# pzimbrod/fem-glass-tempering

Hardware: AMD Instinct MI355X
Metric: DOF-updates/sec (coupled thermo-visco time step, 3D CG1 hex) (higher is better)
Workload: dtype f64; 1 GPU; C4 3D plate CG1/CG1 400x400x50 hex (8200851 T-dofs), dt 0.1, coupled 6-term Prony; parallelism=single GPU, one partition (no communication), output=none (reference writes VTX/XDMF every step), krylov_form=PETSc KSPCG, geometric-multigrid V-cycle preconditioner, preconditioner=gmg, visco_fields=state (T, Tf, Tf_partial, phi, xi, s_tilde, sigma_tilde, sigma)

## Files before the change

fem-glass-tempering_amd/csrc/tv_cg.hip:

```cpp
#include <algorithm>
#include <cstdlib>

#include "tv_stencil.h"


#include <cstdio>
#include <vector>

namespace tv {
namespace {


using buf_t = __amdgpu_buffer_rsrc_t;
using b64v = unsigned int __attribute__((ext_vector_type(2)));
constexpr uint32_t kBadOff = 0x40000000u;
__device__ __forceinline__ buf_t mk_rsrc(const void* p, uint32_t bytes) {
  const uint64_t a = (uint64_t)p;
  const uint32_t lo = __builtin_amdgcn_readfirstlane((uint32_t)a);
  const uint32_t hi = __builtin_amdgcn_readfirstlane((uint32_t)(a >> 32));
  void* q = (void*)(((uint64_t)hi << 32) | lo);
  return __builtin_amdgcn_make_buffer_rsrc(q, (short)0, (int)__builtin_amdgcn_readfirstlane(bytes), 0x00020000);
}
__device__ __forceinline__ double bload(buf_t r, uint32_t off) {
  return __builtin_bit_cast(double, __builtin_amdgcn_raw_buffer_load_b64(r, (int)off, 0, 0));
// ... 274 lines not shown
  double Tp[3][3], Pp[3][3];
#pragma unroll
  for (int u = 0; u < 3; ++u)
#pragma unroll
    for (int v = 0; v < 3; ++v) {
      const int a = c[t1] + u - 1, b = c[t2] + v - 1;
      const bool ok = a >= 0 && a < n[t1] && b >= 0 && b < n[t2];
      const int64_t off = me + (int64_t)(u - 1) * st[t1] + (int64_t)(v - 1) * st[t2];
      if (MODE == MODE_RES) {
        Tp[u][v] = ok ? in0[off] : 0.0;
        Pp[u][v] = 0.0;
      } else {
        Tp[u][v] = ok ? T[off] : 0.0;
        double pv = ok ? in0[off] : 0.0;
        if (FUSEP && ok && !first) pv = pv + bcoef * pold[off];
        Pp[u][v] = pv;
      }
    }
  const double* c1 = g.coef[t1] + (int64_t)c[t1] * C_NCOEF;
  const double* c2 = g.coef[t2] + (int64_t)c[t2] * C_NCOEF;
  return facet_sum<MODE, false, false, false>(g, c1[C_HLO], c1[C_HHI], c2[C_HLO], c2[C_HHI], Tp, Pp);
}

struct FaceOff {
  int off[7];
};

FaceOff face_offsets(const CgGrid& g, int R, int qaxis) {
  FaceOff fo{};
  int acc = 0;
  const int rows = R - 1;
  for (int f = 0; f < 6; ++f) {
    fo.off[f] = acc;
    if (g.fface[f] && (f >> 1) != qaxis) acc += ((g.fn1[f] + kSeg - 1) / kSeg) * ((g.fn2[f] + rows - 1) / rows);
  }
  fo.off[6] = acc;
  return fo;
}

__device__ __forceinline__ void facet_corners(const CgGrid& g, bool ok, double h1, double h2, double Ta,
                                              double Tc, double Pa, double Pc, double& ya, double& yb,
                                              double& yc, double& yd) {
  const double Tb = shl1(Ta), Td = shl1(Tc), Pb = shl1(Pa), Pd = shl1(Pc);
  ya = yb = yc = yd = 0.0;
  if (ok) {
#pragma unroll
    for (int q1 = 0; q1 < 3; ++q1) {
#pragma unroll
      for (int q2 = 0; q2 < 3; ++q2) {
        const double sx = kGX[q1], tx = kGX[q2];
        const double fa = (1.0 - sx) * (1.0 - tx), fb = sx * (1.0 - tx), fc = (1.0 - sx) * tx, fd = sx * tx;
        const double Th = fa * Ta + fb * Tb + fc * Tc + fd * Td;
        const double Ph = fa * Pa + fb * Pb + fc * Pc + fd * Pd;
        const double G = (kGW[q1] * kGW[q2]) * dg_rad_conv(g, Th) * Ph;
        ya += G * fa;
        yb += G * fb;
        yc += G * fc;
        yd += G * fd;
      }
    }
    const double sc = g.dt * (h1 * h2);
    ya *= sc; yb *= sc; yc *= sc; yd *= sc;
  }
}

template <bool FUSEP, int R>
__device__ void face_block(const CgGrid& g, const double* __restrict__ T, const double* __restrict__ in0,
                           const double* pA, const double* pB, double beta_ratio,
                           double* __restrict__ partials, const RedTail& rt, int nrec, int fb,
                           const FaceOff& fo, double* sm, double* redf, int it_host) {
  double (*sT)[kWave] = reinterpret_cast<double (*)[kWave]>(sm);
  double (*sP)[kWave] = reinterpret_cast<double (*)[kWave]>(sm + (R + 1) * kWave);
  double (*sCD)[R][kWave] = reinterpret_cast<double (*)[R][kWave]>(sm + 2 * (R + 1) * kWave);
  int f = 0;
  while (f < 5 && fb >= fo.off[f + 1]) ++f;
  const int a = f >> 1, side = f & 1;
  const int t1 = (a == 0) ? 1 : 0, t2 = (a == 2) ? 1 : 2;
  const int n[3] = {g.n0, g.n1, g.n2};
  const int sst[3] = {1, g.n0, g.n0 * g.n1};
  const int n1 = n[t1], n2 = n[t2];
  const int nseg1 = (n1 + kSeg - 1) / kSeg;
  const int tile = fb - fo.off[f];
  const int seg = tile % nseg1, tb = tile / nseg1;
  const int lane = threadIdx.x & (kWave - 1);
  const int wave = __builtin_amdgcn_readfirstlane(threadIdx.x >> 6);
  const int c1 = seg * kSeg - 1 + lane;
  const int r0 = tb * (R - 1);
// ... 1249 lines not shown
                             hipStream_t s) {
  if (!use_march(g) || !g.bnodes || g.n_bnodes <= 0) return false;
  launch_rows<MODE_RES, false>(g, T, T, Tp, F, nullptr, nullptr, nullptr, false, s, nullptr, 0, true, dinv);
  return true;
}

void launch_cg_japply(const CgGrid& g, const double* T, const double* x, double* y, double* partials,
                      int* n_partials, hipStream_t s, const PcgState* st) {
  launch_rows<MODE_JAC, false>(g, T, x, nullptr, y, nullptr, st, partials, false, s);
  if (n_partials) *n_partials = plan(g, false).nparts;
}

bool launch_cg_japply_tail(const CgGrid& g, const double* T, const double* x, double* y, const PcgState* st,
                           double* partials, const RedTail* tail, hipStream_t s) {
  return launch_rows<MODE_JAC, false>(g, T, x, nullptr, y, nullptr, st, partials, false, s, tail, 0, true);
}

void launch_cg_facet_faces(const CgGrid& g, const double* T, const double* x, const PcgState* st, hipStream_t s) {
  const FaceOff fo = face_offsets(g, kRows, -1);
  if (fo.off[6] <= 0) return;
  hipLaunchKernelGGL(k_cg_faces_all<kRows>, dim3(fo.off[6]), dim3(kRows * kWave), 0, s, g, T, x, fo, st);
}

FaceAdd cg_face_add_all(const CgGrid& g) {
  FaceAdd fa = cg_face_add(g, 0);
  if (!fa.on) return fa;
  for (int f = 0; f < 6; ++f) fa.ff[f] = g.fface[f];
  return fa;
}

void launch_cg_japply_partial(const CgGrid& g, const double* T, const double* x, double* y, const PcgState* st,
                              hipStream_t s) {
  launch_rows<MODE_JAC, false>(g, T, x, nullptr, y, nullptr, st, nullptr, false, s, nullptr, 0, false);
}

bool launch_cg_japply_fused(const CgGrid& g, const double* T, const double* z, double* pA, double* pB,
                            double* w, const PcgState* st, double* partials, int* n_partials,
                            hipStream_t s, const RedTail* tail, int it_host) {
  if (tail && tail->lag && tail->lag_kind != 3) return false;
  const bool fused = launch_rows<MODE_JAC, true>(g, T, z, pA, w, pB, st, partials, true, s, tail, it_host);
  if (n_partials) *n_partials = plan(g, true).nparts;
  return fused;
}

bool launch_cg_cgs(const CgGrid& g, bool init, const CgsBuffers& v, PcgState* st, double* partials,
                   hipStream_t s, const RedTail* tail, int it_host, const double* lag_sums) {
// ... 41 lines not shown
```

fem-glass-tempering_amd/csrc/tv_ctx.h:

```cpp
#pragma once
#include <rccl/rccl.h>

#include <algorithm>
#include <array>
#include <cmath>
#include <cstdio>
#include <cstring>
#include <memory>
#include <mutex>
#include <string>
#include <vector>

#include "tv_internal.h"

namespace tv {

struct FieldInfo {
  double* ptr = nullptr;
  void* base = nullptr;
  int bs = 1;
  int space = 0;
  bool alloc = false;
};

// ... 60 lines not shown
  int64_t globT_off = 0, globS_off = 0;
  int mixed_part = 0;
  int64_t outT_n = 0, outS_n = 0;
  std::vector<std::vector<double>> coords;
  FieldInfo f[TV_NUM_FIELDS];
  double* coef[3] = {nullptr, nullptr, nullptr};
  double* dgh[3] = {nullptr, nullptr, nullptr};
  int* map = nullptr;
  int64_t* bnodes = nullptr;
  double* ffbuf[2] = {nullptr, nullptr};
  double *r = nullptr, *z = nullptr, *pA = nullptr, *pB = nullptr, *w = nullptr, *dinv = nullptr;
  bool cgs = false;
  bool dir_on = false;
  double dir_value = 0.0;
  double *dB = nullptr, *dtmp = nullptr;
  double* Tfo = nullptr;
  int relaxation = TV_RELAX_TAYLOR;
  Output* out = nullptr;
  bool mg_on = false;
  bool mg_dg = false;
  std::vector<MgLevel> mg;
  double mg_omega0 = 0.0;
  double* mgx = nullptr;
  bool mg_cgs = false;
  double* mg_s = nullptr;
  double* dggface = nullptr;
  int mg_A = 0;
  bool mg_local = false;
  double* mg_mask0 = nullptr;
  double* h_big = nullptr;
  size_t h_big_n = 0;
  bool um = false;
  UmGrid umg{};
  std::vector<double> um_xyz;
  std::vector<int64_t> um_cells;
  UmDevice* umd = nullptr;
  unsigned char* um_bmask = nullptr;
  bool amg_on = false;
  std::vector<AmgLevel> amg;
  std::vector<void*> amg_bufs;
  int64_t um_own_cells = 0;
  std::vector<int> um_peer;
  std::vector<int64_t> um_rcnt, um_roff, um_scnt, um_soff;
  int64_t* um_sidx = nullptr;
  double* um_sbuf = nullptr;
  std::vector<int> out_fields;
// ... 120 lines not shown
  int ts_reserve;
  bool ahead;
};
using KrylovIterate = int (*)(void* f, int it, int b, int nb);
using KrylovPublished = int (*)(void* f);
int krylov_drive(Ctx* c, const KrylovPolicy& p, KrylovIterate iterate, void* fi, KrylovPublished published, void* fp,
                 int* its, int* reason);
template <class Iterate, class Published>
int krylov_drive(Ctx* c, const KrylovPolicy& p, Iterate iterate, Published published, int* its, int* reason) {
  return krylov_drive(
      c, p, [](void* f, int it, int b, int nb) -> int { return (*static_cast<Iterate*>(f))(it, b, nb); }, &iterate,
      [](void* f) -> int { return (*static_cast<Published*>(f))(); }, &published, its, reason);
}
CgsBuffers cgs_buffers(Ctx* c, const double* T, int it);
int newton(Ctx* c, int* out_its, int* out_kits, int* out_conv, int step_end = 0, bool* end_queued = nullptr);
int visco(Ctx* c, bool copy_Tprev, const NewtonGate& gate = NewtonGate{});
int queue_newton_norm(Ctx* c, const double* nrm2);
int publish(Ctx* c, void* host_dst, const void* dev_src, size_t bytes);
void launch_bc_mask(Ctx* c, double* dinv);

int mg_setup(Ctx* c);
int mg_prepare(Ctx* c, const double* T);
int mg_dg_weight(Ctx* c, const double* T);
int mg_apply0(Ctx* c, const double* T, const RedTail* tail);
int pcg_solve_mg(Ctx* c, const double* T, int* its, int* reason, bool post = false);
KrylovPolicy mg_krylov_policy(Ctx* c);
bool mg_next_level(const std::vector<double> (&Xp)[3], double da, bool automatic, std::vector<double> (&Xc)[3],
                   std::vector<char> (&is_c)[3], int coarse[3]);
void mg_axis_tables(const std::vector<double>& Xf, const std::vector<char>& is_c, std::vector<int>& pi,
                    std::vector<double>& pw, std::vector<int>& ri, std::vector<double>& rw);
int mg_level_vectors(Ctx* c, MgLevel& L);
double mg_gershgorin(const std::vector<double> (&X)[3], double dt_alpha);
double mg_omega(double b);
int mg_level(Ctx* c, size_t l);
template <class T>
int mg_upload(Ctx* c, MgLevel& L, const std::vector<T>& h, const T** out) {
  void* p = nullptr;
  HIPC(tv_dev_alloc(&p, sizeof(T) * std::max<size_t>(1, h.size()), mem_kind<T>()));
  L.bufs.push_back(p);
  HIPC(hipMemcpy(p, h.data(), sizeof(T) * h.size(), hipMemcpyHostToDevice));
  *out = static_cast<const T*>(p);
  return TV_OK;
}

int mg_setup_dist(Ctx* c);
int pcg_solve_mg_dist(Ctx* c, const double* T, int* its, int* reason, bool post = false);
int mg_prepare_dist(Ctx* c, const double* T);
// ... 5 lines not shown
```

fem-glass-tempering_amd/csrc/tv_internal.h:

```cpp
#pragma once
#include <hip/hip_runtime.h>
#include <cstdint>
#include <string>
#include <type_traits>
#include <vector>

#include "tvfem.h"

namespace tv {

constexpr int kWave = 64;
constexpr int kSeg = kWave - 2;
constexpr int kBlock = 256;

enum { kMemDoubles = 0, kMemOther = 1 };
template <class T>
constexpr int mem_kind() {
  return std::is_same<T, double>::value ? kMemDoubles : kMemOther;
}
hipError_t tv_dev_alloc(void** p, size_t bytes, int kind);
hipError_t tv_dev_free(void* p);
template <class T>
inline hipError_t tv_dev_alloc(T** p, size_t bytes, int kind) {
  void* q = nullptr;
// ... 273 lines not shown
  const double* T_amb;
  const double* eps;
  const int* probes;
  double* hist;
};
void launch_ensemble(const EnsArgs& a, const ViscoConst& c, const ViscoFields& f, const EnsExt* x, hipStream_t s);
void launch_ensemble_dg(const EnsArgs& a, const ViscoConst& c, const ViscoFields& f, const EnsExt* x, hipStream_t s);

constexpr int kVecBlocks = 1024;
constexpr int kVecBlocksMin = 256;
constexpr int kVecNodesPerThread = 16;
constexpr int kVecBlocksMax = 8192;
void launch_pcg_init(int64_t n, const double* r, const double* dinv, double* z, double* dx,
                     double* partials, hipStream_t s);
struct FaceAdd {
  int on;
  int n0, n1, n2;
  int64_t t_off;
  double inv_n0, inv_plane;
  const double* ff[6];
};
FaceAdd cg_face_add(const CgGrid& g, int64_t t_off);


struct MgXfer {
  int fn[3], cn[3];
  int coarse[3];
  int f_kb, f_ke, c_kb, c_ke;
  const int* pi[3];
  const double* pw[3];
  const int* ri[3];
  const double* rw[3];
  int aligned;
};
void launch_mg_restrict(const MgXfer& x, const PcgState* st, const double* bf, const double* wf, const FaceAdd* fa,
                        const double* mask, double* bc, const double* dinv_c, double omega_c, double* xc,
                        hipStream_t s);
struct RRAxis {
  const int* f0;
  const double* w;
};
struct RRArgs {
  int on;
  int fn[3], cn[3];
  RRAxis ax[3];
  double da;
// ... 30 lines not shown
  MgXfer xf[kMgPrepMax];
  double* T[kMgPrepMax];
  double* dinv[kMgPrepMax];
  CgGrid g[kMgPrepMax];
  int64_t off_n[kMgPrepMax + 1];
  int64_t off_b[kMgPrepMax + 1];
};
void launch_mg_prepare(const MgPrep& p, hipStream_t s);
bool cg_uses_march(const CgGrid& g);
void launch_mg_dg_restrict(const DgGrid& g, const PcgState* st, const double* bf, const double* wf, const double* mask,
                           double* bc, const double* dinv_c, double omega_c, double* xc, int kg0, hipStream_t s);
void launch_mg_dg_prolong(const DgGrid& g, const PcgState* st, double* xf, const double* xc, const double* mask,
                          int kg0, hipStream_t s);
void launch_mg_dg_T(const DgGrid& g, const double* Tdg, double* Tcg, int kg0, hipStream_t s);
int launch_mg_pow(int64_t n, const double* dinv, double* y, double* partials, hipStream_t s);
void launch_mg_scale(int64_t n, const double* y, double a, double* x, hipStream_t s);
bool launch_cg_japply_tail(const CgGrid& g, const double* T, const double* x, double* y, const PcgState* st,
                           double* partials, const RedTail* tail, hipStream_t s);
void launch_cg_japply_partial(const CgGrid& g, const double* T, const double* x, double* y, const PcgState* st,
                              hipStream_t s);
void launch_mg_update(int64_t n, const PcgState* st, const double* pA, const double* pB, const double* w,
                      const FaceAdd* fa, const double* dinv, double omega, double* r, double* dx, double* x0,
                      int it_host, int init, hipStream_t s, const double* lag = nullptr,
                      unsigned* counter = nullptr);
void launch_mg_update_cgs(int64_t n, const PcgState* st, const double* u, double* s, const double* z, double* p,
                          double* dx, double* r, const double* dinv, double omega, double* x0, bool first,
                          const double* lag, int lag_kind, unsigned* counter, hipStream_t stream);
int launch_cg_japply_post(const CgGrid& g, const double* T, const double* x, const double* r, const double* dinv,
                          double omega, double* z, const PcgState* st, double* partials, const RedTail* tail,
                          hipStream_t s);
int launch_mg_post(int64_t n, const PcgState* st, const double* x0, const double* r, const double* w,
                   const FaceAdd* fa, const double* dinv, double omega, double* z, double* partials,
                   const RedTail* tail, hipStream_t s);

void launch_pcg_update(int64_t n, PcgState* st, const double* pA, const double* pB, const double* w,
                       const double* dinv, double* dx, double* z, double* partials, hipStream_t s,
                       const RedTail* tail = nullptr, const FaceAdd* fa = nullptr, int it_host = 0);
void launch_pcg_dx_tail(int64_t n, const PcgState* st, const double* pA, const double* pB, double* dx, int its,
                        hipStream_t s);
void launch_mg_dx_finish(int64_t n, const PcgState* st, const double* pA, const double* pB, double* dx, int its,
                         hipStream_t s);
void launch_reduce_logic(const double* partials, int n, int W, double* out, PcgState* st, int kind,
                         int check_done, hipStream_t s);
void launch_logic(PcgState* st, const double* sums, int kind, hipStream_t s);
void launch_set_state(PcgState* st, const PcgState& h, hipStream_t s, const double* gate = nullptr);
void launch_newton_update(int64_t n, double* T, const double* dx, double* partials, hipStream_t s,
                          const RedTail* tail = nullptr);
// ... 22 lines not shown
```

fem-glass-tempering_amd/csrc/tv_mgsolve.cpp:

```cpp
#include <cstdlib>

#include "tv_ctx.h"

namespace tv {
constexpr int64_t kMgFoldFacesNodes = 4000000;

double mg_gershgorin(const std::vector<double> (&X)[3], double dt_alpha) {
  using Row = std::array<double, 6>;
  std::vector<Row> rows[3];
  for (int s = 0; s < 3; ++s) {
    std::vector<double> cf;
    axis_coefs(X[s], 0, (int)X[s].size(), cf);
    for (size_t i = 0; i < X[s].size(); ++i) {
      const double* c = &cf[i * C_NCOEF];
      rows[s].push_back({c[C_MLO], c[C_MDI], c[C_MUP], c[C_KLO], c[C_KDI], c[C_KUP]});
    }
    std::sort(rows[s].begin(), rows[s].end());
    rows[s].erase(std::unique(rows[s].begin(), rows[s].end()), rows[s].end());
  }
  double b = 0.0;
  for (const Row& r0 : rows[0])
    for (const Row& r1 : rows[1])
      for (const Row& r2 : rows[2]) {
        double sum = 0.0, diag = 0.0;
// ... 281 lines not shown
    std::vector<double> rw[3];
    for (int s = 0; s < 3; ++s) {
      std::vector<int> pi;
      std::vector<double> pw;
      mg_axis_tables(Xp[s], is_c[s], pi, pw, ri[s], rw[s]);
      if (int e = mg_upload(c, L, pi, &x.pi[s])) return e;
      if (int e = mg_upload(c, L, pw, &x.pw[s])) return e;
      if (int e = mg_upload(c, L, ri[s], &x.ri[s])) return e;
      if (int e = mg_upload(c, L, rw[s], &x.rw[s])) return e;
      x.fn[s] = (int)Xp[s].size();
      x.cn[s] = (int)L.X[s].size();
      x.coarse[s] = coarse[s];
    }
    x.f_kb = 0;
    x.f_ke = x.fn[2];
    x.c_kb = 0;
    x.c_ke = x.cn[2];
    x.aligned = 1;
    const size_t from = c->mg.size() - 1 - (dg ? 1 : 0);
    if (!dg && ((rr_levels(c->nT) >> from) & 1u))
      if (int e = rr_setup(c, L, Xp, ri, rw)) return e;
    for (int s = 0; s < 3; ++s) Xp[s] = L.X[s];
  }
  c->mg_on = true;
  return TV_OK;
}


int mg_prepare(Ctx* c, const double* T) {
  if (c->amg_on) return TV_OK;
  const bool dgpart = c->mg_dg && c->n_parts > 1;
  auto dg_T = [&](MgLevel& L) -> int {
    if (!dgpart) {
      launch_mg_dg_T(c->dg, T, L.T, 0, c->stream);
      return TV_OK;
    }
    HIPC(hipMemsetAsync(L.T, 0, sizeof(double) * (size_t)L.n, c->stream));
    launch_mg_dg_T(c->dg, T, L.T, c->plane_begin - c->dg.k_begin, c->stream);
    return allreduce_vec(c, L.T, L.n);
  };
  const size_t base = c->mg_dg ? 1 : 0;
  const size_t ncg = c->mg.size() - std::min(c->mg.size(), base);
  bool ready = ncg > 0 && ncg <= (size_t)kMgPrepMax;
  for (size_t l = base; l < c->mg.size() && ready; ++l)
    ready = c->mg[l].dinv_interior && cg_uses_march(c->mg[l].g) && c->mg[l].g.bnodes != nullptr;
  if (ready) {
    if (base == 1) {
      MgLevel& L = c->mg[0];
// ... 50 lines not shown
  if (l < c->mg.size()) {
    const MgLevel& C = c->mg[l];
    const FaceAdd fa = cg_face_add(L.g, 0);
    if (C.rr.on && fa.on) {
      launch_cg_facet_faces(L.g, L.T, L.x, c->st, s);
      if (!launch_mg_rrestrict(C.rr, c->st, L.b, L.x, cg_face_add_all(L.g), C.b, C.dinv, C.omega, C.x, s))
        return c->fail(TV_ERR_STATE, kRRChunkMsg);
    } else if (fa.on && mg_restrict_folds_faces(C.xf)) {
      launch_cg_japply_partial(L.g, L.T, L.x, L.w, c->st, s);
      launch_mg_restrict(C.xf, c->st, L.b, L.w, &fa, nullptr, C.b, C.dinv, C.omega, C.x, s);
    } else {
      launch_cg_japply(L.g, L.T, L.x, L.w, nullptr, nullptr, s, c->st);
      launch_mg_restrict(C.xf, c->st, L.b, L.w, nullptr, nullptr, C.b, C.dinv, C.omega, C.x, s);
    }
    if (int e = mg_level(c, l + 1)) return e;
    mg_prolong_from(c, l, L.x, nullptr);
    launch_cg_japply_partial(L.g, L.T, L.x, L.w, c->st, s);
    if (!mg_prolong_smooths(L.xf))
      launch_mg_jacobi(L.n, c->st, L.b, L.w, &fa, L.dinv, L.omega, L.x, 1, s);
  }
  return TV_OK;
}

int mg_apply0(Ctx* c, const double* T, const RedTail* tail) {
  if (c->amg_on) return amg_apply0(c, tail);
  const int64_t n = c->nT;
  hipStream_t s = c->stream;
  const double* mask = c->dir_on ? c->dinv : nullptr;
  if (c->mg_dg) {
    const DgGrid& d = c->dg;
    MgLevel& C = c->mg[0];
    if (c->n_parts > 1) {
      const int kg0 = c->plane_begin - d.k_begin;
      if (int e = halo(c, c->mgx)) return -e;
      launch_dg_japply(d, T, c->mgx, c->w, nullptr, nullptr, s, c->st);
      if (hipMemsetAsync(C.b, 0, sizeof(double) * (size_t)C.n, s) != hipSuccess)
        return -c->fail(TV_ERR_HIP, "GMG: level-1 memset");
      launch_mg_dg_restrict(d, c->st, c->r, c->w, mask, C.b, nullptr, 0.0, nullptr, kg0, s);
      if (int e = allreduce_vec(c, C.b, C.n)) return -e;
      launch_mg_jacobi(C.n, c->st, C.b, nullptr, nullptr, C.dinv, C.omega, C.x, 0, s);
      if (int e = mg_level(c, 1)) return -e;
      launch_mg_dg_prolong(d, c->st, c->mgx, C.x, mask, kg0, s);
    } else {
      launch_dg_japply(d, T, c->mgx, c->w, nullptr, nullptr, s, c->st);
      launch_mg_dg_restrict(d, c->st, c->r, c->w, mask, C.b, C.dinv, C.omega, C.x, 0, s);
      if (int e = mg_level(c, 1)) return -e;
      launch_mg_dg_prolong(d, c->st, c->mgx, C.x, mask, 0, s);
    }
    launch_dg_japply(d, T, c->mgx, c->w, nullptr, nullptr, s, c->st);
    if (c->dggface)
      return launch_dg_bpost(d, c->st, c->mgx, c->r, c->w, c->dggface, c->mg_omega0, c->z, c->partials, tail, s);
    return launch_mg_post(n, c->st, c->mgx, c->r, c->w, nullptr, c->dinv, c->mg_omega0, c->z, c->partials, tail, s);
  }
  const FaceAdd fa = cg_face_add(c->cg, 0);
  if (!c->mg.empty()) {
    MgLevel& C = c->mg[0];
    if (C.rr.on && mask == nullptr && fa.on) {
      launch_cg_facet_faces(c->cg, T, c->mgx, c->st, s);
      if (!launch_mg_rrestrict(C.rr, c->st, c->r, c->mgx, cg_face_add_all(c->cg), C.b, C.dinv, C.omega, C.x, s))
        return -c->fail(TV_ERR_STATE, kRRChunkMsg);
    } else if (fa.on && mg_restrict_folds_faces(C.xf) && n < kMgFoldFacesNodes) {
      launch_cg_japply_partial(c->cg, T, c->mgx, c->w, c->st, s);
      launch_mg_restrict(C.xf, c->st, c->r, c->w, &fa, mask, C.b, C.dinv, C.omega, C.x, s);
    } else {
      launch_cg_japply(c->cg, T, c->mgx, c->w, nullptr, nullptr, s, c->st);
      launch_mg_restrict(C.xf, c->st, c->r, c->w, nullptr, mask, C.b, C.dinv, C.omega, C.x, s);
    }
    if (int e = mg_level(c, 1)) return -e;
    mg_prolong_from(c, 0, c->mgx, mask);
  }
  {
    const int nrec = launch_cg_japply_post(c->cg, T, c->mgx, c->r, c->dinv, c->mg_omega0, c->z, c->st, c->partials,
                                           tail, s);
    if (nrec >= 0) return nrec;
  }
  launch_cg_japply_partial(c->cg, T, c->mgx, c->w, c->st, s);
  return launch_mg_post(n, c->st, c->mgx, c->r, c->w, &fa, c->dinv, c->mg_omega0, c->z, c->partials, tail, s);
}

int mg_iteration(Ctx* c, const double* T, int it) {
  const int64_t n = c->nT;
  RedTail t1{c->counters, c->partials, c->sums, c->st, 2, iter_stamp(c, it)};
  int np = 0;
  if (!op_japply_fused(c, T, &np, &t1, it))
    if (int e = reduce_logic(c, np, 1, 2, 1)) return e;
  const FaceAdd fa = (c->mg_dg || c->um) ? FaceAdd{} : cg_face_add(c->cg, 0);
  if (c->dggface)
    launch_dg_bupdate(c->dg, c->st, c->pA, c->pB, c->w, c->dggface, c->mg_omega0, c->r, c->f[TV_F_DX].ptr, c->mgx, it, 0,
                      c->stream);
  else
    launch_mg_update(n, c->st, c->pA, c->pB, c->w, &fa, c->dinv, c->mg_omega0, c->r, c->f[TV_F_DX].ptr, c->mgx, it, 0,
                     c->stream);
  RedTail t2{c->counters + kTailCounters, c->partials, c->sums, c->st, 3, nullptr};
  const int nrec = mg_apply0(c, T, &t2);
  return nrec < 0 ? -nrec : TV_OK;
}

KrylovPolicy mg_krylov_policy(Ctx* c) {
  KrylovPolicy p{};
  p.ahead = false;
  p.hints = c->mg_hint;
  p.hint_min = 0;
  p.first_default = 1;
  p.hint_floor = 1;
  p.next = 1;
  p.guard = c->O.ksp_max_it + 2;
  p.ts_reserve = c->O.ksp_max_it + 8;
  return p;
}

int pcg_solve_mg(Ctx* c, const double* T, int* its, int* reason, bool post) {
  const int64_t n = c->nT;
  solve_begin(c, c->solve_gate);
  if (int e = mg_prepare(c, T)) return e;
  if (int e = mg_dg_weight(c, T)) return e;
  if (c->dggface)
    launch_dg_bupdate(c->dg, c->st, c->pA, c->pB, c->w, c->dggface, c->mg_omega0, c->r, c->f[TV_F_DX].ptr, c->mgx, 0, 1,
                      c->stream);
  else
    launch_mg_update(n, c->st, c->pA, c->pB, c->w, nullptr, c->dinv, c->mg_omega0, c->r, c->f[TV_F_DX].ptr, c->mgx, 0, 1,
                     c->stream);
  RedTail t0{c->counters + kTailCounters, c->partials, c->sums, c->st, 1, nullptr};
  if (const int nrec = mg_apply0(c, T, &t0); nrec < 0) return -nrec;
  auto iterate = [&](int it, int, int) { return mg_iteration(c, T, it); };
  auto published = [&]() -> int {
    if (!post) return TV_OK;
    launch_post_group(n, c->st, c->pA, c->pB, c->f[TV_F_DX].ptr, c->f[TV_F_T].ptr, c->partials, c->sums, c->stream);
    return queue_newton_norm(c, c->sums);
  };
  if (int e = krylov_drive(c, mg_krylov_policy(c), iterate, published, its, reason)) return e;
  if (!post) launch_mg_dx_finish(n, c->st, c->pA, c->pB, c->f[TV_F_DX].ptr, *its, c->stream);
  return TV_OK;
}

}

using namespace tv;

static int precond_apply_part(Ctx* c, const double* r_dev, double* z_dev) {
  if (int e = require_comm(c, "tv_precond_apply")) return e;
  if (c->um || c->fam_T != TV_CG) return c->fail(TV_ERR_ARG, "tv_precond_apply: partitioned CG1 box meshes");
  const double* T = c->f[TV_F_T].ptr;
  const int64_t off = c->ownT_off, n = c->ownT_n;
  hipStream_t s = c->stream;
  if (int e = halo(c, c->f[TV_F_T].ptr)) return e;
  launch_cg_diag(c->cg, T, c->dinv, 1, s, c->dinv_interior);
// ... 4 lines not shown
  } else {
    PcgState h{};
    HIPC(hipMemcpyAsync(c->st, &h, sizeof(PcgState), hipMemcpyHostToDevice, s));
    if (int e = mg_prepare_dist(c, T)) return e;
    if (c->dir_on)
      if (int e = halo(c, c->dinv)) return e;
    if (c->mg_mask0) launch_mg_ownmask(c->nT, off, off + n, c->dir_on ? c->dinv : nullptr, c->mg_mask0, s);
    HIPC(hipMemcpyAsync(c->r + off, r_dev, sizeof(double) * (size_t)n, hipMemcpyDeviceToDevice, s));
    int64_t woff, nwin;
    fine_window(c, &woff, &nwin);
    if (c->ghost_depth > 1)
      if (int e = halo(c, c->r)) return e;
    launch_mg_jacobi(nwin, c->st, c->r + woff, nullptr, nullptr, c->dinv + woff, c->mg_omega0, c->mgx + woff, 0, s);
    if (int e = mg_apply0_dist(c, T, nullptr)) return e;
    HIPC(hipMemcpyAsync(z_dev, c->z + off, sizeof(double) * (size_t)n, hipMemcpyDeviceToDevice, s));
  }
  HIPC(hipGetLastError());
  HIPC(hipStreamSynchronize(s));
  return TV_OK;
}

extern "C" {

int tv_precond_apply(void* ctx, const double* r_dev, double* z_dev) {
  Ctx* c = static_cast<Ctx*>(ctx);
  if (!c || !r_dev || !z_dev) return TV_ERR_ARG;
  hipSetDevice(c->device);
  HIPC(hipDeviceSynchronize());
  if (c->n_parts > 1) return precond_apply_part(c, r_dev, z_dev);
  const double* T = c->f[TV_F_T].ptr;
  const int64_t n = c->nT;
  hipStream_t s = c->stream;
  if (!c->dggface) {
    if (!c->um && c->fam_T == TV_CG) {
      launch_cg_diag(c->cg, T, c->dinv, 1, s, c->dinv_interior);
      c->dinv_interior = true;
    } else {
      op_diag(c, T, c->dinv, 1);
    }
  }
  if (c->dir_on && c->fam_T == TV_CG) launch_bc_mask(c, c->dinv);
  if (c->mg_dg || c->amg_on)
    if (int e = mg_dg_weight(c, T)) return e;
  if (!c->mg_on) {
    launch_mg_jacobi(n, nullptr, r_dev, nullptr, nullptr, c->dinv, 1.0, z_dev, 0, s);
  } else {
// ... 18 lines not shown
```

fem-glass-tempering_amd/csrc/tv_pcg.hip:

```cpp
#include <algorithm>
#include <cstdlib>

#include "tv_device.h"

namespace tv {
namespace {

__device__ __forceinline__ double wave_sum(double v) {
#pragma unroll
  for (int off = 32; off >= 1; off >>= 1) v += __shfl_xor(v, off, 64);
  return v;
}

template <int W>
__device__ __forceinline__ void block_partials(double (&v)[W], double* partials) {
  __shared__ double red[W][kBlock / kWave];
  const int lane = threadIdx.x & 63, wave = threadIdx.x >> 6;
#pragma unroll
  for (int w = 0; w < W; ++w) {
    const double s = wave_sum(v[w]);
    if (lane == 0) red[w][wave] = s;
  }
  __syncthreads();
  if (threadIdx.x < W) {
    const int w = threadIdx.x;
    store_partial(&partials[(int64_t)blockIdx.x * W + w], (red[w][0] + red[w][1]) + (red[w][2] + red[w][3]));
// ... 66 lines not shown
      v[4] = ldc<NT1>(&pp[q]);
      v[5] = p[q];
    }
  };
  constexpr int U = 4;
  const int64_t stride = (int64_t)gridDim.x * kBlock;
  int64_t t = blockIdx.x * (int64_t)kBlock + threadIdx.x;
  for (; t + (U - 1) * stride < n; t += U * stride) {
    double v[U][6];
#pragma unroll
    for (int u = 0; u < U; ++u) load(t + u * stride, v[u]);
#pragma unroll
    for (int u = 0; u < U; ++u) node(t + u * stride, v[u]);
  }
  for (; t < n; t += stride) {
    double v[6];
    load(t, v);
    node(t, v);
  }
  block_partials<2>(acc, partials);
  fused_reduce_tail<2>(rt, gridDim.x);
}

template <bool FACES, bool INIT, bool DXU, bool FIRST = false>
__global__ __launch_bounds__(kBlock) void k_mg_update(int64_t n, const PcgState* __restrict__ st,
                                                      const double* __restrict__ pA, const double* __restrict__ pB,
                                                      const double* __restrict__ w, FaceAdd fa,
                                                      const double* __restrict__ dinv, double omega,
                                                      double* __restrict__ r, double* __restrict__ dx,
                                                      double* __restrict__ x0, int it_host, const double* lag,
                                                      unsigned* counter, PcgState* st_w) {
  double a = 0.0, ap = 0.0;
  if (!INIT && lag != nullptr) {
    const PcgState ls = lagged_state(st, lag, 2);
    if (ls.done) { commit_done(st_w, ls); return; }
    a = ls.a;
    ap = DXU ? ls.a_prev : 0.0;
  } else {
    if (st->done) return;
    a = INIT ? 0.0 : st->a;
    ap = DXU ? st->a_prev : 0.0;
  }
  const double* __restrict__ p = (it_host & 1) ? pB : pA;
  const double* __restrict__ pp = (it_host & 1) ? pA : pB;
  auto load = [&](int64_t q, double (&v)[6]) {
    v[0] = r[q];
    v[2] = ldc<true>(&dinv[q]);
    if (!INIT) v[1] = ldc<true>(&w[q]);
    if (DXU) {
      v[3] = FIRST ? 0.0 : ldc<true>(&dx[q]);
      v[4] = ldc<true>(&pp[q]);
      v[5] = ldc<true>(&p[q]);
    }
  };
  auto node = [&](int64_t q, const double (&v)[6]) {
    double rr = v[0];
    if (INIT) {
    } else {
      double wt = v[1];
      if (FACES) wt += face_terms(fa, q);
      rr -= a * wt;
      r[q] = rr;
      if (DXU) stc<true>(&dx[q], (v[3] + ap * v[4]) + a * v[5]);
    }
    x0[q] = omega * v[2] * rr;
  };
  constexpr int U = 4;
  const int64_t stride = (int64_t)gridDim.x * kBlock;
  int64_t t = blockIdx.x * (int64_t)kBlock + threadIdx.x;
  for (; t + (U - 1) * stride < n; t += U * stride) {
    double v[U][6];
#pragma unroll
    for (int u = 0; u < U; ++u) load(t + u * stride, v[u]);
#pragma unroll
    for (int u = 0; u < U; ++u) node(t + u * stride, v[u]);
  }
  for (; t < n; t += stride) {
    double v[6];
    load(t, v);
    node(t, v);
  }
  if (!INIT && lag != nullptr && last_block_arrived(counter, gridDim.x) && threadIdx.x == 0) {
    const PcgState ls = lagged_state(st, lag, 2);
    *st_w = ls;
  }
}

template <bool FIRST>
__global__ __launch_bounds__(kBlock) void k_mg_update_cgs(int64_t n, const PcgState* __restrict__ st,
                                                          const double* __restrict__ u, double* __restrict__ s,
                                                          const double* __restrict__ z, double* __restrict__ p,
                                                          double* __restrict__ dx, double* __restrict__ r,
// ... 174 lines not shown
__global__ __launch_bounds__(kBlock) void k_copy(double* __restrict__ d, const double* __restrict__ s, int64_t n) {
  for (int64_t t = blockIdx.x * (int64_t)kBlock + threadIdx.x; t < n; t += (int64_t)gridDim.x * kBlock) d[t] = s[t];
}

int vec_blocks(int64_t n) {
  int64_t b = (n + kBlock - 1) / kBlock;
  const int64_t lim = std::min<int64_t>(kVecBlocks, std::max<int64_t>(kVecBlocksMin,
      (n + (int64_t)kBlock * kVecNodesPerThread - 1) / ((int64_t)kBlock * kVecNodesPerThread)));
  if (b > lim) b = lim;
  return b < 1 ? 1 : (int)b;
}

}

int pcg_vec_blocks(int64_t n) { return vec_blocks(n); }

void launch_pcg_init(int64_t n, const double* r, const double* dinv, double* z, double* dx, double* partials,
                     hipStream_t s) {
  hipLaunchKernelGGL(k_pcg_init, dim3(vec_blocks(n)), dim3(kBlock), 0, s, n, r, dinv, z, dx, partials);
}

void launch_mg_update(int64_t n, const PcgState* st, const double* pA, const double* pB, const double* w,
                      const FaceAdd* fa, const double* dinv, double omega, double* r, double* dx, double* x0,
                      int it_host, int init, hipStream_t s, const double* lag, unsigned* counter) {
  const FaceAdd f = (fa && fa->on) ? *fa : FaceAdd{};
  const dim3 g(vec_blocks(n)), b(kBlock);
  const bool odd = (it_host & 1) != 0;
  const bool first = it_host == 1;
#define TV_MGU(F, I, D, FI) \
  hipLaunchKernelGGL((k_mg_update<F, I, D, FI>), g, b, 0, s, n, st, pA, pB, w, f, dinv, omega, r, dx, x0, it_host, \
                     lag, counter, const_cast<PcgState*>(st))
  if (init) TV_MGU(false, true, false, false);
  else if (f.on) {
    if (first) TV_MGU(true, false, true, true);
    else if (odd) TV_MGU(true, false, true, false);
    else TV_MGU(true, false, false, false);
  } else {
    if (first) TV_MGU(false, false, true, true);
    else if (odd) TV_MGU(false, false, true, false);
    else TV_MGU(false, false, false, false);
  }
#undef TV_MGU
}

int launch_mg_post(int64_t n, const PcgState* st, const double* x0, const double* r, const double* w,
                   const FaceAdd* fa, const double* dinv, double omega, double* z, double* partials,
                   const RedTail* tail, hipStream_t s) {
  const RedTail rt = tail ? *tail : RedTail{};
  const FaceAdd f = (fa && fa->on) ? *fa : FaceAdd{};
  const int nb = vec_blocks(n);
  if (f.on)
    hipLaunchKernelGGL(k_mg_post<true>, dim3(nb), dim3(kBlock), 0, s, n, st, x0, r, w, f, dinv, omega, z, partials, rt);
  else
    hipLaunchKernelGGL(k_mg_post<false>, dim3(nb), dim3(kBlock), 0, s, n, st, x0, r, w, f, dinv, omega, z, partials, rt);
// ... 98 lines not shown
```

fem-glass-tempering_amd/csrc/tv_stencil.h:

```cpp
#pragma once
#include "tv_device.h"

namespace tv {
namespace {

enum { MODE_RES = 0, MODE_JAC = 1 };

__device__ constexpr double kGX[3] = {0.11270166537925831148, 0.5, 0.88729833462074168852};
__device__ constexpr double kGW[3] = {5.0 / 18.0, 8.0 / 18.0, 5.0 / 18.0};

__device__ __forceinline__ double g_rad_conv(const CgGrid& g, double T) {
  const double T2 = T * T;
  return g.a_rad * (T2 * T2 - g.T_amb4) + g.a_conv * (T - g.T_amb);
}
__device__ __forceinline__ double dg_rad_conv(const CgGrid& g, double T) {
  return g.a_rad * 4.0 * (T * T * T) + g.a_conv;
}

template <int MODE, bool DIAG, bool D1, bool D2>
__device__ double facet_sum(const CgGrid& g, double h1lo, double h1hi, double h2lo, double h2hi,
                            const double (&Tp)[3][3], const double (&Pp)[3][3]) {
  double acc = 0.0;
  constexpr int NS1 = D1 ? 1 : 2, NQ1 = D1 ? 1 : 3;
  constexpr int NS2 = D2 ? 1 : 2, NQ2 = D2 ? 1 : 3;
#pragma unroll
  for (int s1 = 0; s1 < NS1; ++s1) {
    const double h1 = D1 ? 1.0 : (s1 == 0 ? h1lo : h1hi);
    if (!D1 && !(h1 > 0.0)) continue;
    const int o1 = D1 ? 0 : (s1 == 0 ? -1 : 1);
#pragma unroll
    for (int s2 = 0; s2 < NS2; ++s2) {
      const double h2 = D2 ? 1.0 : (s2 == 0 ? h2lo : h2hi);
      if (!D2 && !(h2 > 0.0)) continue;
      const int o2 = D2 ? 0 : (s2 == 0 ? -1 : 1);
      const double T00 = Tp[1][1], T10 = Tp[1 + o1][1], T01 = Tp[1][1 + o2], T11 = Tp[1 + o1][1 + o2];
      const double P00 = Pp[1][1], P10 = Pp[1 + o1][1], P01 = Pp[1][1 + o2], P11 = Pp[1 + o1][1 + o2];
#pragma unroll
      for (int q1 = 0; q1 < NQ1; ++q1) {
        const double pc1 = D1 ? 1.0 : (s1 == 0 ? kGX[q1] : 1.0 - kGX[q1]);
// ... 65 lines not shown
```

Baseline: 846.7 million DOF-updates/s.

## Fold boundary-facet Jacobian of x0 into the MG update kernel

Extra blocks are appended to the multigrid update kernel. Each one recomputes the updated residual and the Jacobi x0 on boundary faces and evaluates the radiation/convection facet contribution of x0 into a face buffer. This removes the separate launch_cg_facet_faces kernel and its reread of r, dinv and T on the faces before restriction. It caches face residuals, dinv and T in double-buffered face arrays, adds four face-sized allocations, and duplicates the residual update on face nodes.

```diff
diff --git a/fem-glass-tempering_amd/csrc/tv_cg.hip b/fem-glass-tempering_amd/csrc/tv_cg.hip
--- a/fem-glass-tempering_amd/csrc/tv_cg.hip
+++ b/fem-glass-tempering_amd/csrc/tv_cg.hip
@@ -320,10 +320,6 @@
   return facet_sum<MODE, false, false, false>(g, c1[C_HLO], c1[C_HHI], c2[C_HLO], c2[C_HHI], Tp, Pp);
 }
 
-struct FaceOff {
-  int off[7];
-};
-
 FaceOff face_offsets(const CgGrid& g, int R, int qaxis) {
   FaceOff fo{};
   int acc = 0;
@@ -336,31 +332,6 @@
   return fo;
 }
 
-__device__ __forceinline__ void facet_corners(const CgGrid& g, bool ok, double h1, double h2, double Ta,
-                                              double Tc, double Pa, double Pc, double& ya, double& yb,
-                                              double& yc, double& yd) {
-  const double Tb = shl1(Ta), Td = shl1(Tc), Pb = shl1(Pa), Pd = shl1(Pc);
-  ya = yb = yc = yd = 0.0;
-  if (ok) {
-#pragma unroll
-    for (int q1 = 0; q1 < 3; ++q1) {
-#pragma unroll
-      for (int q2 = 0; q2 < 3; ++q2) {
-        const double sx = kGX[q1], tx = kGX[q2];
-        const double fa = (1.0 - sx) * (1.0 - tx), fb = sx * (1.0 - tx), fc = (1.0 - sx) * tx, fd = sx * tx;
-        const double Th = fa * Ta + fb * Tb + fc * Tc + fd * Td;
-        const double Ph = fa * Pa + fb * Pb + fc * Pc + fd * Pd;
-        const double G = (kGW[q1] * kGW[q2]) * dg_rad_conv(g, Th) * Ph;
-        ya += G * fa;
-        yb += G * fb;
-        yc += G * fc;
-        yd += G * fd;
-      }
-    }
-    const double sc = g.dt * (h1 * h2);
-    ya *= sc; yb *= sc; yc *= sc; yd *= sc;
-  }
-}
 
 template <bool FUSEP, int R>
 __device__ void face_block(const CgGrid& g, const double* __restrict__ T, const double* __restrict__ in0,
@@ -1656,6 +1627,8 @@
   hipLaunchKernelGGL(k_cg_faces_all<kRows>, dim3(fo.off[6]), dim3(kRows * kWave), 0, s, g, T, x, fo, st);
 }
 
+FaceOff cg_face_offsets_all(const CgGrid& g, int R) { return face_offsets(g, R, -1); }
+
 FaceAdd cg_face_add_all(const CgGrid& g) {
   FaceAdd fa = cg_face_add(g, 0);
   if (!fa.on) return fa;
diff --git a/fem-glass-tempering_amd/csrc/tv_ctx.h b/fem-glass-tempering_amd/csrc/tv_ctx.h
--- a/fem-glass-tempering_amd/csrc/tv_ctx.h
+++ b/fem-glass-tempering_amd/csrc/tv_ctx.h
@@ -106,6 +106,8 @@
   std::vector<MgLevel> mg;
   double mg_omega0 = 0.0;
   double* mgx = nullptr;
+  double* rfbuf[4] = {nullptr, nullptr, nullptr, nullptr};
+  bool mg_fold_ok = false, mg_fold = false;
   bool mg_cgs = false;
   double* mg_s = nullptr;
   double* dggface = nullptr;
@@ -272,7 +274,7 @@
 int mg_setup(Ctx* c);
 int mg_prepare(Ctx* c, const double* T);
 int mg_dg_weight(Ctx* c, const double* T);
-int mg_apply0(Ctx* c, const double* T, const RedTail* tail);
+int mg_apply0(Ctx* c, const double* T, const RedTail* tail, bool x0_faces = false);
 int pcg_solve_mg(Ctx* c, const double* T, int* its, int* reason, bool post = false);
 KrylovPolicy mg_krylov_policy(Ctx* c);
 bool mg_next_level(const std::vector<double> (&Xp)[3], double da, bool automatic, std::vector<double> (&Xc)[3],
diff --git a/fem-glass-tempering_amd/csrc/tv_internal.h b/fem-glass-tempering_amd/csrc/tv_internal.h
--- a/fem-glass-tempering_amd/csrc/tv_internal.h
+++ b/fem-glass-tempering_amd/csrc/tv_internal.h
@@ -319,6 +319,23 @@
 };
 FaceAdd cg_face_add(const CgGrid& g, int64_t t_off);
 
+struct FaceOff {
+  int off[7];
+};
+FaceOff cg_face_offsets_all(const CgGrid& g, int R);
+
+struct MgFold {
+  int on;
+  CgGrid g;
+  const double* T;
+  FaceOff fo;
+  const double* rold[6];
+  double* rnew[6];
+  double* xface[6];
+  double* tface[6];
+  double* dface[6];
+};
+
 
 struct MgXfer {
   int fn[3], cn[3];
@@ -395,7 +412,7 @@
 void launch_mg_update(int64_t n, const PcgState* st, const double* pA, const double* pB, const double* w,
                       const FaceAdd* fa, const double* dinv, double omega, double* r, double* dx, double* x0,
                       int it_host, int init, hipStream_t s, const double* lag = nullptr,
-                      unsigned* counter = nullptr);
+                      unsigned* counter = nullptr, const MgFold* fold = nullptr);
 void launch_mg_update_cgs(int64_t n, const PcgState* st, const double* u, double* s, const double* z, double* p,
                           double* dx, double* r, const double* dinv, double omega, double* x0, bool first,
                           const double* lag, int lag_kind, unsigned* counter, hipStream_t stream);
diff --git a/fem-glass-tempering_amd/csrc/tv_mgsolve.cpp b/fem-glass-tempering_amd/csrc/tv_mgsolve.cpp
--- a/fem-glass-tempering_amd/csrc/tv_mgsolve.cpp
+++ b/fem-glass-tempering_amd/csrc/tv_mgsolve.cpp
@@ -327,8 +327,41 @@
       if (int e = rr_setup(c, L, Xp, ri, rw)) return e;
     for (int s = 0; s < 3; ++s) Xp[s] = L.X[s];
   }
+  const char* fe = std::getenv("TVFEM_MG_FOLD");
+  const bool fold_env = !(fe && std::atoi(fe) == 0);
+  if (!dg && fold_env && c->n_parts == 1 && !c->mg.empty() && c->mg[0].rr.on && cg_face_add(c->cg, 0).on &&
+      c->cg.ffsize > 0 && c->cg.ffbuf[1] != nullptr) {
+    for (int q = 0; q < 4; ++q) {
+      void* p = nullptr;
+      HIPC(tv_dev_alloc(&p, sizeof(double) * (size_t)c->cg.ffsize, kMemDoubles));
+      HIPC(hipMemsetAsync(p, 0, sizeof(double) * (size_t)c->cg.ffsize, c->stream));
+      c->mg[0].bufs.push_back(p);
+      c->rfbuf[q] = static_cast<double*>(p);
+    }
+    c->mg_fold_ok = true;
+  }
   c->mg_on = true;
   return TV_OK;
+}
+
+static MgFold mg_fold_args(Ctx* c, const double* T, int it, bool init) {
+  MgFold m{};
+  if (!c->mg_fold) return m;
+  m.on = 1;
+  m.g = c->cg;
+  m.T = T;
+  m.fo = cg_face_offsets_all(c->cg, kBlock / kWave);
+  const int ro = init ? 0 : (it & 1), wn = init ? 0 : ((it + 1) & 1);
+  for (int f = 0; f < 6; ++f) {
+    const int64_t off = c->cg.ffoff[f];
+    if (off < 0 || !c->cg.fface[f]) continue;
+    m.rold[f] = c->rfbuf[ro] + off;
+    m.rnew[f] = c->rfbuf[wn] + off;
+    m.xface[f] = c->cg.ffbuf[1] + off;
+    m.tface[f] = c->rfbuf[2] + off;
+    m.dface[f] = c->rfbuf[3] + off;
+  }
+  return m;
 }
 
 
@@ -425,7 +458,7 @@
   return TV_OK;
 }
 
-int mg_apply0(Ctx* c, const double* T, const RedTail* tail) {
+int mg_apply0(Ctx* c, const double* T, const RedTail* tail, bool x0_faces) {
   if (c->amg_on) return amg_apply0(c, tail);
   const int64_t n = c->nT;
   hipStream_t s = c->stream;
@@ -459,8 +492,14 @@
   if (!c->mg.empty()) {
     MgLevel& C = c->mg[0];
     if (C.rr.on && mask == nullptr && fa.on) {
-      launch_cg_facet_faces(c->cg, T, c->mgx, c->st, s);
-      if (!launch_mg_rrestrict(C.rr, c->st, c->r, c->mgx, cg_face_add_all(c->cg), C.b, C.dinv, C.omega, C.x, s))
+      FaceAdd fx = cg_face_add_all(c->cg);
+      if (x0_faces) {
+        for (int f = 0; f < 6; ++f)
+          if (fx.ff[f]) fx.ff[f] = c->cg.ffbuf[1] + c->cg.ffoff[f];
+      } else {
+        launch_cg_facet_faces(c->cg, T, c->mgx, c->st, s);
+      }
+      if (!launch_mg_rrestrict(C.rr, c->st, c->r, c->mgx, fx, C.b, C.dinv, C.omega, C.x, s))
         return -c->fail(TV_ERR_STATE, kRRChunkMsg);
     } else if (fa.on && mg_restrict_folds_faces(C.xf) && n < kMgFoldFacesNodes) {
       launch_cg_japply_partial(c->cg, T, c->mgx, c->w, c->st, s);
@@ -491,11 +530,13 @@
   if (c->dggface)
     launch_dg_bupdate(c->dg, c->st, c->pA, c->pB, c->w, c->dggface, c->mg_omega0, c->r, c->f[TV_F_DX].ptr, c->mgx, it, 0,
                       c->stream);
-  else
+  else {
+    const MgFold fold = mg_fold_args(c, T, it, false);
     launch_mg_update(n, c->st, c->pA, c->pB, c->w, &fa, c->dinv, c->mg_omega0, c->r, c->f[TV_F_DX].ptr, c->mgx, it, 0,
-                     c->stream);
+                     c->stream, nullptr, nullptr, &fold);
+  }
   RedTail t2{c->counters + kTailCounters, c->partials, c->sums, c->st, 3, nullptr};
-  const int nrec = mg_apply0(c, T, &t2);
+  const int nrec = mg_apply0(c, T, &t2, c->mg_fold);
   return nrec < 0 ? -nrec : TV_OK;
 }
 
@@ -517,14 +558,17 @@
   solve_begin(c, c->solve_gate);
   if (int e = mg_prepare(c, T)) return e;
   if (int e = mg_dg_weight(c, T)) return e;
+  c->mg_fold = c->mg_fold_ok && !c->dir_on && !c->amg_on && !c->mg_dg;
   if (c->dggface)
     launch_dg_bupdate(c->dg, c->st, c->pA, c->pB, c->w, c->dggface, c->mg_omega0, c->r, c->f[TV_F_DX].ptr, c->mgx, 0, 1,
                       c->stream);
-  else
+  else {
+    const MgFold fold = mg_fold_args(c, T, 0, true);
     launch_mg_update(n, c->st, c->pA, c->pB, c->w, nullptr, c->dinv, c->mg_omega0, c->r, c->f[TV_F_DX].ptr, c->mgx, 0, 1,
-                     c->stream);
+                     c->stream, nullptr, nullptr, &fold);
+  }
   RedTail t0{c->counters + kTailCounters, c->partials, c->sums, c->st, 1, nullptr};
-  if (const int nrec = mg_apply0(c, T, &t0); nrec < 0) return -nrec;
+  if (const int nrec = mg_apply0(c, T, &t0, c->mg_fold); nrec < 0) return -nrec;
   auto iterate = [&](int it, int, int) { return mg_iteration(c, T, it); };
   auto published = [&]() -> int {
     if (!post) return TV_OK;
@@ -575,6 +619,14 @@
 
 extern "C" {
 
+int tv_mg_update_faces(void* ctx, int* in_force, int* set_up) {
+  Ctx* c = static_cast<Ctx*>(ctx);
+  if (!c || !in_force || !set_up) return TV_ERR_ARG;
+  *in_force = c->mg_fold ? 1 : 0;
+  *set_up = c->mg_fold_ok ? 1 : 0;
+  return TV_OK;
+}
+
 int tv_precond_apply(void* ctx, const double* r_dev, double* z_dev) {
   Ctx* c = static_cast<Ctx*>(ctx);
   if (!c || !r_dev || !z_dev) return TV_ERR_ARG;
diff --git a/fem-glass-tempering_amd/csrc/tv_pcg.hip b/fem-glass-tempering_amd/csrc/tv_pcg.hip
--- a/fem-glass-tempering_amd/csrc/tv_pcg.hip
+++ b/fem-glass-tempering_amd/csrc/tv_pcg.hip
@@ -1,7 +1,7 @@
 #include <algorithm>
 #include <cstdlib>
 
-#include "tv_device.h"
+#include "tv_stencil.h"
 
 namespace tv {
 namespace {
@@ -114,14 +114,101 @@
   fused_reduce_tail<2>(rt, gridDim.x);
 }
 
-template <bool FACES, bool INIT, bool DXU, bool FIRST = false>
+
+__device__ __forceinline__ double mg_update_r(double r, double a, double wt) { return __builtin_fma(-a, wt, r); }
+__device__ __forceinline__ double mg_update_x0(double omega, double dinv, double r) { return omega * dinv * r; }
+
+template <bool FOLD>
+struct MgFoldArg {
+  MgFold m;
+};
+template <>
+struct MgFoldArg<false> {};
+constexpr int kFoldR = kBlock / kWave;
+constexpr int kFoldLds = (2 * (kFoldR + 1) + 2 * kFoldR) * kWave;
+template <bool INIT>
+__device__ void mg_update_face_block(const MgFold& m, const FaceAdd& fa, double a, double omega,
+                                     const double* __restrict__ r, const double* __restrict__ w,
+                                     const double* __restrict__ dinv, int fb, double* sm) {
+  constexpr int R = kFoldR;
+  const CgGrid& g = m.g;
+  double (*sT)[kWave] = reinterpret_cast<double (*)[kWave]>(sm);
+  double (*sP)[kWave] = reinterpret_cast<double (*)[kWave]>(sm + (R + 1) * kWave);
+  double (*sCD)[R][kWave] = reinterpret_cast<double (*)[R][kWave]>(sm + 2 * (R + 1) * kWave);
+  int f = 0;
+  while (f < 5 && fb >= m.fo.off[f + 1]) ++f;
+  const int ax = f >> 1, side = f & 1;
+  const int t1 = (ax == 0) ? 1 : 0, t2 = (ax == 2) ? 1 : 2;
+  const int n[3] = {g.n0, g.n1, g.n2};
+  const int n1 = n[t1], n2 = n[t2];
+  const int nseg1 = (n1 + kSeg - 1) / kSeg;
+  const int tile = fb - m.fo.off[f];
+  const int seg = tile % nseg1, tb = tile / nseg1;
+  const int lane = threadIdx.x & (kWave - 1);
+  const int wave = __builtin_amdgcn_readfirstlane(threadIdx.x >> 6);
+  const int c1 = seg * kSeg - 1 + lane;
+  const int r0 = tb * (R - 1);
+  const bool ok1 = c1 >= 0 && c1 < n1;
+  const double* __restrict__ rold = m.rold[f];
+  double keep_d = 0.0, keep_t = 0.0;
+  auto stage = [&](int row, int cc2) -> double {
+    const bool ok = ok1 && cc2 >= 0 && cc2 < n2;
+    int c[3];
+    c[t1] = ok ? c1 : 0;
+    c[t2] = ok ? cc2 : 0;
+    c[ax] = side ? n[ax] - 1 : 0;
+    const int64_t o = c[0] + (int64_t)n[0] * (c[1] + (int64_t)n[1] * c[2]);
+    const int64_t e = c[t1] + (int64_t)n1 * c[t2];
+    double rr = INIT ? r[o] : rold[e];
+    const double di = INIT ? dinv[o] : m.dface[f][e], tt = INIT ? m.T[o] : m.tface[f][e];
+    if (INIT && row == wave) {
+      keep_d = di;
+      keep_t = tt;
+    }
+    if (!INIT) {
+      double wt = w[o];
+      wt += face_at(fa, c[0], c[1], c[2]);
+      rr = mg_update_r(rr, a, wt);
+    }
+    sT[row][lane] = ok ? tt : 0.0;
+    sP[row][lane] = ok ? mg_update_x0(omega, di, rr) : 0.0;
+    return rr;
+  };
+  const int fr = r0 - 1 + wave;
+  const bool facet_ok = c1 >= 0 && c1 < n1 - 1 && fr >= 0 && fr < n2 - 1;
+  const double h1 = g.coef[t1][(int64_t)(facet_ok ? c1 : 0) * C_NCOEF + C_HHI];
+  const double h2 = g.coef[t2][(int64_t)(facet_ok ? fr : 0) * C_NCOEF + C_HHI];
+  const double rn = stage(wave, fr);
+  if (wave == R - 1) stage(R, r0 + R - 1);
+  __syncthreads();
+  double ya, yb, yc, yd;
+  facet_corners(g, facet_ok, h1, h2, sT[wave][lane], sT[wave + 1][lane], sP[wave][lane], sP[wave + 1][lane], ya, yb,
+                yc, yd);
+  sCD[0][wave][lane] = yc;
+  sCD[1][wave][lane] = yd;
+  const double ybl = shr1(yb);
+  __syncthreads();
+  const int c2 = fr;
+  if (wave >= 1 && ok1 && lane >= 1 && lane <= kSeg && c2 < n2) {
+    const double acc = (ya + ybl) + (sCD[0][wave - 1][lane] + sCD[1][wave - 1][lane - 1]);
+    const int64_t e = c1 + (int64_t)n1 * c2;
+    m.xface[f][e] = acc;
+    m.rnew[f][e] = rn;
+    if (INIT) {
+      m.dface[f][e] = keep_d;
+      m.tface[f][e] = keep_t;
+    }
+  }
+}
+
+template <bool FACES, bool INIT, bool DXU, bool FIRST = false, bool FOLD = false>
 __global__ __launch_bounds__(kBlock) void k_mg_update(int64_t n, const PcgState* __restrict__ st,
                                                       const double* __restrict__ pA, const double* __restrict__ pB,
                                                       const double* __restrict__ w, FaceAdd fa,
                                                       const double* __restrict__ dinv, double omega,
                                                       double* __restrict__ r, double* __restrict__ dx,
                                                       double* __restrict__ x0, int it_host, const double* lag,
-                                                      unsigned* counter, PcgState* st_w) {
+                                                      unsigned* counter, PcgState* st_w, MgFoldArg<FOLD> fold) {
   double a = 0.0, ap = 0.0;
   if (!INIT && lag != nullptr) {
     const PcgState ls = lagged_state(st, lag, 2);
@@ -133,6 +220,17 @@
     a = INIT ? 0.0 : st->a;
     ap = DXU ? st->a_prev : 0.0;
   }
+  int nface = 0;
+  const int bid = (int)blockIdx.x;
+  if constexpr (FOLD) {
+    __shared__ double fsm[kFoldLds];
+    nface = fold.m.fo.off[6];
+    const int fb = bid - ((int)gridDim.x - nface);
+    if (fb >= 0) {
+      mg_update_face_block<INIT>(fold.m, fa, a, omega, r, w, dinv, fb, fsm);
+      return;
+    }
+  }
   const double* __restrict__ p = (it_host & 1) ? pB : pA;
   const double* __restrict__ pp = (it_host & 1) ? pA : pB;
   auto load = [&](int64_t q, double (&v)[6]) {
@@ -151,15 +249,15 @@
     } else {
       double wt = v[1];
       if (FACES) wt += face_terms(fa, q);
-      rr -= a * wt;
+      rr = mg_update_r(rr, a, wt);
       r[q] = rr;
       if (DXU) stc<true>(&dx[q], (v[3] + ap * v[4]) + a * v[5]);
     }
-    x0[q] = omega * v[2] * rr;
+    x0[q] = mg_update_x0(omega, v[2], rr);
   };
   constexpr int U = 4;
-  const int64_t stride = (int64_t)gridDim.x * kBlock;
-  int64_t t = blockIdx.x * (int64_t)kBlock + threadIdx.x;
+  const int64_t stride = (int64_t)((int)gridDim.x - nface) * kBlock;
+  int64_t t = bid * (int64_t)kBlock + threadIdx.x;
   for (; t + (U - 1) * stride < n; t += U * stride) {
     double v[U][6];
 #pragma unroll
@@ -380,14 +478,30 @@
 
 void launch_mg_update(int64_t n, const PcgState* st, const double* pA, const double* pB, const double* w,
                       const FaceAdd* fa, const double* dinv, double omega, double* r, double* dx, double* x0,
-                      int it_host, int init, hipStream_t s, const double* lag, unsigned* counter) {
+                      int it_host, int init, hipStream_t s, const double* lag, unsigned* counter,
+                      const MgFold* fold) {
   const FaceAdd f = (fa && fa->on) ? *fa : FaceAdd{};
-  const dim3 g(vec_blocks(n)), b(kBlock);
+  const dim3 b(kBlock);
   const bool odd = (it_host & 1) != 0;
   const bool first = it_host == 1;
+  if (fold && fold->on && fold->fo.off[6] > 0 && lag == nullptr && (init || f.on)) {
+    const dim3 g(fold->fo.off[6] + vec_blocks(n));
+    const MgFoldArg<true> fo{*fold};
+#define TV_MGUF(F, I, D, FI) \
+  hipLaunchKernelGGL((k_mg_update<F, I, D, FI, true>), g, b, 0, s, n, st, pA, pB, w, f, dinv, omega, r, dx, x0, \
+                     it_host, lag, counter, const_cast<PcgState*>(st), fo)
+    if (init) TV_MGUF(false, true, false, false);
+    else if (first) TV_MGUF(true, false, true, true);
+    else if (odd) TV_MGUF(true, false, true, false);
+    else TV_MGUF(true, false, false, false);
+#undef TV_MGUF
+    return;
+  }
+  const dim3 g(vec_blocks(n));
+  const MgFoldArg<false> nofold{};
 #define TV_MGU(F, I, D, FI) \
   hipLaunchKernelGGL((k_mg_update<F, I, D, FI>), g, b, 0, s, n, st, pA, pB, w, f, dinv, omega, r, dx, x0, it_host, \
-                     lag, counter, const_cast<PcgState*>(st))
+                     lag, counter, const_cast<PcgState*>(st), nofold)
   if (init) TV_MGU(false, true, false, false);
   else if (f.on) {
     if (first) TV_MGU(true, false, true, true);
diff --git a/fem-glass-tempering_amd/csrc/tv_stencil.h b/fem-glass-tempering_amd/csrc/tv_stencil.h
--- a/fem-glass-tempering_amd/csrc/tv_stencil.h
+++ b/fem-glass-tempering_amd/csrc/tv_stencil.h
@@ -15,6 +15,32 @@
 }
 __device__ __forceinline__ double dg_rad_conv(const CgGrid& g, double T) {
   return g.a_rad * 4.0 * (T * T * T) + g.a_conv;
+}
+
+__device__ __forceinline__ void facet_corners(const CgGrid& g, bool ok, double h1, double h2, double Ta,
+                                              double Tc, double Pa, double Pc, double& ya, double& yb,
+                                              double& yc, double& yd) {
+  const double Tb = shl1(Ta), Td = shl1(Tc), Pb = shl1(Pa), Pd = shl1(Pc);
+  ya = yb = yc = yd = 0.0;
+  if (ok) {
+#pragma unroll
+    for (int q1 = 0; q1 < 3; ++q1) {
+#pragma unroll
+      for (int q2 = 0; q2 < 3; ++q2) {
+        const double sx = kGX[q1], tx = kGX[q2];
+        const double fa = (1.0 - sx) * (1.0 - tx), fb = sx * (1.0 - tx), fc = (1.0 - sx) * tx, fd = sx * tx;
+        const double Th = fa * Ta + fb * Tb + fc * Tc + fd * Td;
+        const double Ph = fa * Pa + fb * Pb + fc * Pc + fd * Pd;
+        const double G = (kGW[q1] * kGW[q2]) * dg_rad_conv(g, Th) * Ph;
+        ya += G * fa;
+        yb += G * fb;
+        yc += G * fc;
+        yd += G * fd;
+      }
+    }
+    const double sc = g.dt * (h1 * h2);
+    ya *= sc; yb *= sc; yc *= sc; yd *= sc;
+  }
 }
 
 template <int MODE, bool DIAG, bool D1, bool D2>
```

New measurement: 851.2 million DOF-updates/s, median of 3. About the same (+0.5%).
